# chenxing1999/recsys-benchmark

Hardware: AMD Instinct MI355X
Metric: samples/sec fwd+bwd, Criteo-26field DeepFM b=4096; HBM GB/s vs roofline (higher is better)
Workload: dtype f32; 1 GPU; C2 DeepFM Criteo-26field full embedding: F=26, D=16, N=33762577 rows, MLP 400x3+BN+dropout0.5, B=4096/GPU, fwd+bwd, 16 distinct uniform-id batches rotated (fresh ids every step), row-form (COO) table grads, criterion evaluated in the head launch (model(x, labels=y)), next batch known one step ahead (its table rows touched by riders of the weight-gradient launch), tables stored as one packed [N,32]; global_batch=4096, parallelism=single

## Files before the change

### recsys-benchmark_amd/csrc/tail.hip

```cpp
#include <cstdlib>
#include <type_traits>

#include "common.hpp"
#include "tail_gemm.hpp"
#include "tail_masks.hpp"

namespace {
using namespace mi;
using namespace tg;

__device__ __forceinline__ Drop make_drop(const uint8_t *bits, float p, int ld) {
  Drop d;
  d.bits = p > 0.f ? bits : nullptr;
  d.inv_keep = p > 0.f ? 1.f / (1.f - p) : 1.f;
  d.ld = ld;
  return d;
}

__global__ __launch_bounds__(kBlock) void k_tail_dropmask(MaskJob j, const int64_t *seed, float4 *__restrict__ zero4, int64_t nzero4) {
  mask_blocks(j, seed, zero4, nzero4, blockIdx.x, gridDim.x);
}

constexpr int kTilePitch = BNT + 4;
__device__ __forceinline__ void acc_to_lds(const floatx4 (&acc)[NSUB], const floatx4 (&accg)[NGRP], Cover cv, float *T, int wave,
// ... 473 lines not shown
  const float rstd = rsqrtf(var + eps);
  mu[n] = mean_a;
  sc[n] = gm * rstd;
  be[n] = bt;
  rstd_out[n] = rstd;
  if (running_mean) {
    running_mean[n] = (1.f - momentum) * rm + momentum * (mean_a + mo);
    const float unb = M > 1 ? m2_a / (float)(M - 1) : var;
    running_var[n] = (1.f - momentum) * rv + momentum * unb;
  }
}

template <bool MERGE>
__global__ __launch_bounds__(kBlock) void k_tail_head_fwd(ActDesc x, const float *__restrict__ w, const float *__restrict__ b,
                                                          const float *__restrict__ add, float *__restrict__ out, int M,
                                                          int N, BnFwd bn, int64_t *bump) {
  __shared__ __attribute__((aligned(16))) float cst[MERGE ? 3 * kCstPitch : 4];
  if (bump && blockIdx.x == 0 && threadIdx.x == 0) bump[0] += 1;
  const int lane = threadIdx.x & 63;
  const int wave0 = blockIdx.x * kWavesPerBlock + (threadIdx.x >> 6), nw = gridDim.x * kWavesPerBlock;
  const float bv = b ? b[0] : 0.f;
  auto rows = [&](const auto &act, const auto &between) {
    if (N <= 512) {
      const int c0 = lane * 4, c1 = lane * 4 + 256;
      const bool v0 = c0 < N, v1 = c1 < N;
      const float4 w0 = v0 ? ld4(w + c0) : make_float4(0.f, 0.f, 0.f, 0.f), w1 = v1 ? ld4(w + c1) : make_float4(0.f, 0.f, 0.f, 0.f);
      bool first = true;
      for (int m0 = wave0; m0 < M || first; m0 += 4 * nw) {
        typename std::remove_reference<decltype(act)>::type::Raw r0[4], r1[4];
        if (m0 < M) {
#pragma unroll
          for (int u = 0; u < 4; ++u) {
            const int m = min(m0 + u * nw, M - 1);
            if (v0) r0[u] = act.fetch(m, c0);
            if (v1) r1[u] = act.fetch(m, c1);
          }
        }
        if (first) between();
        first = false;
        if (m0 >= M) break;
#pragma unroll
        for (int u = 0; u < 4; ++u) {
          const int m = m0 + u * nw;
          if (m >= M) break;
          float s = 0.f;
          if (v0) { const float4 a = act.finish(r0[u], act.consts(c0), m, c0); s += a.x * w0.x + a.y * w0.y + a.z * w0.z + a.w * w0.w; }
          if (v1) { const float4 a = act.finish(r1[u], act.consts(c1), m, c1); s += a.x * w1.x + a.y * w1.y + a.z * w1.z + a.w * w1.w; }
          s = wave_sum(s);
          if (lane == 0) out[m] = s + bv + (add ? add[m] : 0.f);
        }
      }
      return;
    }
    between();
    for (int m = wave0; m < M; m += nw) {
      float s = 0.f;
      for (int c = lane * 4; c < N; c += 256) {
        const float4 a = act.finish(act.fetch(m, c), act.consts(c), m, c), ww = ld4(w + c);
        s += a.x * ww.x + a.y * ww.y + a.z * ww.z + a.w * ww.w;
      }
      s = wave_sum(s);
      if (lane == 0) out[m] = s + bv + (add ? add[m] : 0.f);
    }
  };
  const LoadAct act = make_act(x);
  if constexpr (MERGE) {
    const lds_cfp c = as_lds(cst);
    rows(LoadActL{x.Z, x.ld, c, c + kCstPitch, c + 2 * kCstPitch, act.drop}, [&]() {
      bn_merge_fwd<kBlock>(bn, M, N, cst, blockIdx.x == 0, (int)threadIdx.x);
      __syncthreads();
    });
  } else {
    rows(act, []() {});
  }
}

constexpr int kHeadRows = 8;
__global__ __launch_bounds__(kBlock) void k_tail_head_bwd(ActDesc x, const float *__restrict__ g, const float *__restrict__ w,
                                                          float *__restrict__ DY, float *__restrict__ part,
                                                          float *__restrict__ wpart, int M, int N, int reps) {
  const Drop drop = make_drop(x.keep, x.p, x.ld);
  const int c = threadIdx.x * 4;
  const bool cv = c < N;
  float4 s_dy = zero4(), s_dyz = zero4(), s_ga = zero4();
  float s_g = 0.f;
  float4 u_ = zero4(), sc = zero4(), be = zero4(), ww = zero4();
  if (cv) { u_ = ld4(x.mu + c); sc = ld4(x.sc + c); be = ld4(x.be + c); ww = ld4(w + c); }
  const int rows_per = (M + gridDim.x - 1) / gridDim.x;
  const int mb = blockIdx.x * rows_per, me = min(M, mb + rows_per);
  for (int m4 = mb; m4 < me; m4 += kHeadRows) {
    float4 z[kHeadRows];
    uint32_t kb[kHeadRows];
    float gv[kHeadRows];
#pragma unroll
    for (int u = 0; u < kHeadRows; ++u) {
      const int m = min(m4 + u, me - 1);
      gv[u] = g[m];
      if (cv) {
        z[u] = ld4(x.Z + (int64_t)m * x.ld + c);
        kb[u] = drop.fetch(m, c);
      }
    }
    loads_landed();
#pragma unroll
    for (int u = 0; u < kHeadRows; ++u) {
      const int m = m4 + u;
      if (m >= me) break;
      const float gm = gv[u];
      s_g += gm;
      if (!cv) continue;
      const float4 k = drop.scale4(kb[u], c);
      const float4 zc = make_float4(z[u].x - u_.x, z[u].y - u_.y, z[u].z - u_.z, z[u].w - u_.w);
      const float4 pre = make_float4(fmaf(zc.x, sc.x, be.x), fmaf(zc.y, sc.y, be.y), fmaf(zc.z, sc.z, be.z), fmaf(zc.w, sc.w, be.w));
      float4 dy;
      dy.x = pre.x > 0.f ? gm * ww.x * k.x : 0.f;
      dy.y = pre.y > 0.f ? gm * ww.y * k.y : 0.f;
      dy.z = pre.z > 0.f ? gm * ww.z * k.z : 0.f;
      dy.w = pre.w > 0.f ? gm * ww.w * k.w : 0.f;
      st4(DY + (int64_t)m * x.ld + c, dy);
      s_dy.x += dy.x; s_dy.y += dy.y; s_dy.z += dy.z; s_dy.w += dy.w;
      s_dyz.x += dy.x * zc.x; s_dyz.y += dy.y * zc.y; s_dyz.z += dy.z * zc.z; s_dyz.w += dy.w * zc.w;
      s_ga.x += gm * fmaxf(pre.x, 0.f) * k.x; s_ga.y += gm * fmaxf(pre.y, 0.f) * k.y;
      s_ga.z += gm * fmaxf(pre.z, 0.f) * k.z; s_ga.w += gm * fmaxf(pre.w, 0.f) * k.w;
    }
  }
  if (reps > 0) {
    __shared__ float sp[2 * 4 * kBlock + 4 * kBlock + 4];
    float *sw = sp + 2 * 4 * kBlock;
    if (cv) {
      st4(sp + c * 2, make_float4(s_dy.x, s_dyz.x, s_dy.y, s_dyz.y));
      st4(sp + c * 2 + 4, make_float4(s_dy.z, s_dyz.z, s_dy.w, s_dyz.w));
      st4(sw + c, s_ga);
    }
    if (threadIdx.x == 0) sw[N] = s_g;
    lds_barrier();
    const int rr = blockIdx.x % reps;
    float *o = part + (int64_t)rr * N * 2;
    for (int i = threadIdx.x; i < 2 * N; i += kBlock) atomicAdd(o + i, sp[i]);
    float *q = wpart + (int64_t)rr * (N + 4);
    for (int i = threadIdx.x; i <= N; i += kBlock) atomicAdd(q + i, sw[i]);
    return;
  }
  if (cv) {
    float *o = part + ((int64_t)blockIdx.x * N + c) * 2;
    st4(o, make_float4(s_dy.x, s_dyz.x, s_dy.y, s_dyz.y));
    st4(o + 4, make_float4(s_dy.z, s_dyz.z, s_dy.w, s_dyz.w));
    st4(wpart + (int64_t)blockIdx.x * (N + 4) + c, s_ga);
  }
  if (threadIdx.x == 0) wpart[(int64_t)blockIdx.x * (N + 4) + N] = s_g;
}

constexpr int kHeadLossCols = 512;
constexpr int kHeadLossRed = 3 * kHeadLossCols + 4;
template <int MERGE>
__global__ __launch_bounds__(kBlock) void k_tail_head_bce(ActDesc x, const float *__restrict__ w, const float *__restrict__ b,
                                                          const float *__restrict__ add, const float *__restrict__ y,
                                                          float *__restrict__ out, float *__restrict__ gout,
                                                          float *__restrict__ DY, float *__restrict__ part,
                                                          float *__restrict__ wpart, float *__restrict__ loss_ws, int M,
                                                          int N, BnFwd bn, int reps, int64_t *bump,
                                                          const float *__restrict__ upstream) {
  __shared__ __attribute__((aligned(16))) float cst[MERGE != 0 ? 3 * kCstPitch : 4];
  __shared__ __attribute__((aligned(16))) float red[kWavesPerBlock][kHeadLossRed];
  if (bump && blockIdx.x == 0 && threadIdx.x == 0) bump[0] += 1;
  const int lane = threadIdx.x & 63, wv = __builtin_amdgcn_readfirstlane(threadIdx.x >> 6);
  const int wave0 = blockIdx.x * kWavesPerBlock + wv, nw = gridDim.x * kWavesPerBlock;
  const Drop drop = make_drop(x.keep, x.p, x.ld);
  const float bv = b ? b[0] : 0.f;
  const float inv_m = 1.f / (float)M;
  const float gsc = upstream ? upstream[0] * inv_m : inv_m;
  const int c0 = lane * 4, c1 = lane * 4 + 256;
  const bool v0 = c0 < N, v1 = c1 < N;
  const float4 w0 = v0 ? ld4(w + c0) : zero4(), w1 = v1 ? ld4(w + c1) : zero4();
  float4 mu0 = zero4(), sc0 = zero4(), be0 = zero4(), mu1 = zero4(), sc1 = zero4(), be1 = zero4();
  float4 dy0 = zero4(), dz0 = zero4(), ga0 = zero4(), dy1 = zero4(), dz1 = zero4(), ga1 = zero4();
  float s_g = 0.f, s_loss = 0.f;
  bool first = true;
  for (int m0 = wave0; m0 < M || first; m0 += 4 * nw) {
    float4 z0[4], z1[4];
    uint32_t k0[4], k1[4];
    float av[4], yv[4];
    if (m0 < M) {
#pragma unroll
      for (int u = 0; u < 4; ++u) {
        const int m = min(m0 + u * nw, M - 1);
        if (v0) { z0[u] = ld4(x.Z + (int64_t)m * x.ld + c0); k0[u] = drop.fetch(m, c0); }
        if (v1) { z1[u] = ld4(x.Z + (int64_t)m * x.ld + c1); k1[u] = drop.fetch(m, c1); }
        av[u] = add ? add[m] : 0.f;
        yv[u] = y[m];
      }
    }
    if (first) {
      if constexpr (MERGE != 0) {
        if constexpr (MERGE == 2) bn_derive_fwd<kBlock>(bn, M, N, cst, blockIdx.x == 0, (int)threadIdx.x);
        else bn_merge_fwd<kBlock>(bn, M, N, cst, blockIdx.x == 0, (int)threadIdx.x);
        __syncthreads();
        const lds_cfp c = as_lds(cst);
        if (v0) { mu0 = vld4(c + c0); sc0 = vld4(c + kCstPitch + c0); be0 = vld4(c + 2 * kCstPitch + c0); }
        if (v1) { mu1 = vld4(c + c1); sc1 = vld4(c + kCstPitch + c1); be1 = vld4(c + 2 * kCstPitch + c1); }
      } else {
        if (v0) { mu0 = ld4(x.mu + c0); sc0 = ld4(x.sc + c0); be0 = ld4(x.be + c0); }
        if (v1) { mu1 = ld4(x.mu + c1); sc1 = ld4(x.sc + c1); be1 = ld4(x.be + c1); }
      }
    }
    first = false;
    loads_landed();
    if (m0 >= M) break;
    float sa[4];
    auto row0 = [&](int u, float4 &zc, float4 &pre, float4 &kk) {
      kk = drop.scale4(k0[u], c0);
      zc = make_float4(z0[u].x - mu0.x, z0[u].y - mu0.y, z0[u].z - mu0.z, z0[u].w - mu0.w);
      pre = make_float4(fmaf(zc.x, sc0.x, be0.x), fmaf(zc.y, sc0.y, be0.y), fmaf(zc.z, sc0.z, be0.z), fmaf(zc.w, sc0.w, be0.w));
    };
    auto row1 = [&](int u, float4 &zc, float4 &pre, float4 &kk) {
      kk = drop.scale4(k1[u], c1);
      zc = make_float4(z1[u].x - mu1.x, z1[u].y - mu1.y, z1[u].z - mu1.z, z1[u].w - mu1.w);
      pre = make_float4(fmaf(zc.x, sc1.x, be1.x), fmaf(zc.y, sc1.y, be1.y), fmaf(zc.z, sc1.z, be1.z), fmaf(zc.w, sc1.w, be1.w));
    };
#pragma unroll
    for (int u = 0; u < 4; ++u) {
      float4 zc, pre, kk;
      float s = 0.f;
      if (v0) {
        row0(u, zc, pre, kk);
        s += fmaxf(pre.x, 0.f) * kk.x * w0.x + fmaxf(pre.y, 0.f) * kk.y * w0.y + fmaxf(pre.z, 0.f) * kk.z * w0.z +
             fmaxf(pre.w, 0.f) * kk.w * w0.w;
      }
      if (v1) {
        row1(u, zc, pre, kk);
        s += fmaxf(pre.x, 0.f) * kk.x * w1.x + fmaxf(pre.y, 0.f) * kk.y * w1.y + fmaxf(pre.z, 0.f) * kk.z * w1.z +
             fmaxf(pre.w, 0.f) * kk.w * w1.w;
      }
      sa[u] = s;
    }
#pragma unroll
    for (int msk = 32; msk >= 1; msk >>= 1) {
#pragma unroll
      for (int u = 0; u < 4; ++u) sa[u] += __shfl_xor(sa[u], msk);
    }
    float4 d0[4], d1[4];
    float xo[4], go[4];
#pragma unroll
    for (int u = 0; u < 4; ++u) {
      const int m = m0 + u * nw;
      if (m >= M) break;
      float4 zc0 = zero4(), zc1 = zero4(), pre0 = zero4(), pre1 = zero4(), kk0 = zero4(), kk1 = zero4();
      if (v0) row0(u, zc0, pre0, kk0);
      if (v1) row1(u, zc1, pre1, kk1);
      const float s = sa[u];
      const float xl = s + bv + av[u];
      const float gm = gsc * (1.f / (1.f + expf(-xl)) - yv[u]);
      s_loss += fmaxf(xl, 0.f) - xl * yv[u] + log1pf(expf(-fabsf(xl)));
      s_g += gm;
      xo[u] = xl; go[u] = gm;
      if (v0) {
        float4 d;
        d.x = pre0.x > 0.f ? gm * w0.x * kk0.x : 0.f;
        d.y = pre0.y > 0.f ? gm * w0.y * kk0.y : 0.f;
        d.z = pre0.z > 0.f ? gm * w0.z * kk0.z : 0.f;
        d.w = pre0.w > 0.f ? gm * w0.w * kk0.w : 0.f;
        d0[u] = d;
        dy0.x += d.x; dy0.y += d.y; dy0.z += d.z; dy0.w += d.w;
        dz0.x += d.x * zc0.x; dz0.y += d.y * zc0.y; dz0.z += d.z * zc0.z; dz0.w += d.w * zc0.w;
        ga0.x += gm * fmaxf(pre0.x, 0.f) * kk0.x; ga0.y += gm * fmaxf(pre0.y, 0.f) * kk0.y;
        ga0.z += gm * fmaxf(pre0.z, 0.f) * kk0.z; ga0.w += gm * fmaxf(pre0.w, 0.f) * kk0.w;
      }
      if (v1) {
        float4 d;
        d.x = pre1.x > 0.f ? gm * w1.x * kk1.x : 0.f;
        d.y = pre1.y > 0.f ? gm * w1.y * kk1.y : 0.f;
        d.z = pre1.z > 0.f ? gm * w1.z * kk1.z : 0.f;
        d.w = pre1.w > 0.f ? gm * w1.w * kk1.w : 0.f;
        d1[u] = d;
        dy1.x += d.x; dy1.y += d.y; dy1.z += d.z; dy1.w += d.w;
        dz1.x += d.x * zc1.x; dz1.y += d.y * zc1.y; dz1.z += d.z * zc1.z; dz1.w += d.w * zc1.w;
        ga1.x += gm * fmaxf(pre1.x, 0.f) * kk1.x; ga1.y += gm * fmaxf(pre1.y, 0.f) * kk1.y;
        ga1.z += gm * fmaxf(pre1.z, 0.f) * kk1.z; ga1.w += gm * fmaxf(pre1.w, 0.f) * kk1.w;
      }
    }
#pragma unroll
    for (int u = 0; u < 4; ++u) {
      const int m = m0 + u * nw;
      if (m >= M) break;
      if (lane == 0) { out[m] = xo[u]; gout[m] = go[u]; }
      if (v0) st4(DY + (int64_t)m * x.ld + c0, d0[u]);
      if (v1) st4(DY + (int64_t)m * x.ld + c1, d1[u]);
    }
  }
  float *rp = red[wv];
  if (v0) {
    st4(rp + 2 * c0, make_float4(dy0.x, dz0.x, dy0.y, dz0.y));
    st4(rp + 2 * c0 + 4, make_float4(dy0.z, dz0.z, dy0.w, dz0.w));
    st4(rp + 2 * kHeadLossCols + c0, ga0);
  }
  if (v1) {
    st4(rp + 2 * c1, make_float4(dy1.x, dz1.x, dy1.y, dz1.y));
    st4(rp + 2 * c1 + 4, make_float4(dy1.z, dz1.z, dy1.w, dz1.w));
    st4(rp + 2 * kHeadLossCols + c1, ga1);
  }
  if (lane == 0) { rp[3 * kHeadLossCols] = s_g; rp[3 * kHeadLossCols + 1] = s_loss; }
  lds_barrier();
  const int rr = blockIdx.x % reps;
  constexpr int kSumThreads = kBlock - kWave;
  if (wv < kWavesPerBlock - 1) {
    float *o = part + (int64_t)rr * N * 2;
    for (int i = threadIdx.x; i < 2 * N; i += kSumThreads) atomicAdd(o + i, (red[0][i] + red[1][i]) + (red[2][i] + red[3][i]));
    float *q = wpart + (int64_t)rr * (N + 4);
    for (int i = threadIdx.x; i <= N; i += kSumThreads) {
      const int j = i < N ? 2 * kHeadLossCols + i : 3 * kHeadLossCols;
      atomicAdd(q + i, (red[0][j] + red[1][j]) + (red[2][j] + red[3][j]));
    }
  } else {
    if (lane == 0) {
      const int j = 3 * kHeadLossCols + 1;
      const float lp = ((red[0][j] + red[1][j]) + (red[2][j] + red[3][j])) * inv_m;
      atomicAdd(loss_ws + 4 + rr, lp);
      __threadfence();
      const uint32_t mine = ((uint32_t)gridDim.x - (uint32_t)rr + (uint32_t)reps - 1u) / (uint32_t)reps;
      const uint32_t old = atomicAdd(reinterpret_cast<uint32_t *>(loss_ws + 4 + reps) + rr, 1u);
      if (old == mine - 1u) {
        __threadfence();
        const float v = __hip_atomic_load(loss_ws + 4 + rr, __ATOMIC_RELAXED, __HIP_MEMORY_SCOPE_AGENT);
        atomicAdd(loss_ws, v);
      }
    }
    loads_landed();
  }
}

__global__ __launch_bounds__(kBlock) void k_bn_finalize_bwd(const float *__restrict__ part, int nblk, int M, int N,
                                                            const float *__restrict__ gamma, const float *__restrict__ rstd,
                                                            float *__restrict__ dgamma, float *__restrict__ dbeta,
                                                            float *__restrict__ al, float *__restrict__ bz,
                                                            float *__restrict__ de, const float *__restrict__ wpart,
                                                            int nwblk, float *__restrict__ dw, float *__restrict__ db,
                                                            int affine, float *__restrict__ dbias, float *__restrict__ db2) {
  __shared__ float sh[kFinGroups][kFinCols][3];
  const int cl = threadIdx.x % kFinCols, grp = threadIdx.x / kFinCols;
  const int n = blockIdx.x * kFinCols + cl;
  float r = 0.f, gm = 1.f;
  if (grp == 0 && n < N) { r = rstd[n]; if (gamma) gm = gamma[n]; }
  float s1 = 0.f, s2 = 0.f, sw = 0.f;
  if (n < N) {
    const int per = (nblk + kFinGroups - 1) / kFinGroups, t0 = grp * per, t1 = min(nblk, t0 + per);
    for (int base = t0; base < t1; base += 16) {
      float2 v[16];
#pragma unroll
      for (int u = 0; u < 16; ++u) v[u] = *reinterpret_cast<const float2 *>(part + ((int64_t)min(base + u, t1 - 1) * N + n) * 2);
#pragma unroll
      for (int u = 0; u < 16; ++u)
        if (base + u < t1) { s1 += v[u].x; s2 += v[u].y; }
    }
  }
  if (wpart && n <= N) {
    const int per = (nwblk + kFinGroups - 1) / kFinGroups, t0 = grp * per, t1 = min(nwblk, t0 + per);
    for (int base = t0; base < t1; base += 16) {
      float v[16];
#pragma unroll
      for (int u = 0; u < 16; ++u) v[u] = wpart[(int64_t)min(base + u, t1 - 1) * (N + 4) + n];
#pragma unroll
      for (int u = 0; u < 16; ++u)
        if (base + u < t1) sw += v[u];
    }
  }
  sh[grp][cl][0] = s1; sh[grp][cl][1] = s2; sh[grp][cl][2] = sw;
  __syncthreads();
  if (grp != 0 || n > N) return;
  s1 = 0.f; s2 = 0.f; sw = 0.f;
#pragma unroll
  for (int q = 0; q < kFinGroups; ++q) { s1 += sh[q][cl][0]; s2 += sh[q][cl][1]; sw += sh[q][cl][2]; }
  if (wpart) {
    if (n < N) dw[n] = sw;
    else {
      if (db) db[0] = sw;
      if (db2) db2[0] = sw;
    }
  }
  if (n >= N) return;
  const float dg = s2 * r;
  if (dgamma) dgamma[n] = dg;
  if (dbeta) dbeta[n] = s1;
  const float inv_m = 1.f / (float)M;
  al[n] = gm * r;
  bz[n] = affine ? 0.f : -gm * r * r * dg * inv_m;
  de[n] = affine ? 0.f : -gm * r * s1 * inv_m;
  if (affine && dbias) dbias[n] = gm * r * s1;
}

__global__ __launch_bounds__(kBlock) void k_tail_affine_consts(AffineJob j) {
  affine_consts_blocks(j, (int)blockIdx.x, (int)gridDim.x);
}

struct DgradArgs {
  DzDesc dz;
  const float *W;
  int ldw;
  ActDesc prev;
  float *OUT;
  int ldo;
  float *part;
  int part_rep;
  float *dz_out;
  int M, N, K;
  int ncols, ntn;
  BnBwd bn;
  const float *fm_emb;
  const float *fm_sum;
  const float *fm_gy;
  float *fm_g1;
  int fm_D;
  const int64_t *fm_slot;
  int fm_pitch;
};

template <bool DZ, bool MID, bool MERGE, bool FM = false>
__global__ __launch_bounds__(kThreads) void k_tail_dgrad(DgradArgs a) {
  __shared__ __attribute__((aligned(16))) float lds[kLdsFloats + (MERGE ? kCstFloats : 0)];
  const int mt_total = (a.M + BM - 1) / BM;
  const int tile = xcd_logical(blockIdx.x, mt_total * a.ntn);
  if (tile < 0) return;

  const int mt = tile / a.ntn, nt = tile % a.ntn;
  const int m0 = mt * BM, k0 = nt * a.ncols;
  const int rows_valid = min(BM, a.M - m0), cols_valid = min(a.ncols, a.K - k0);
  const int lane = threadIdx.x & 63, wave = threadIdx.x >> 6;
  floatx4 acc[NSUB], accg[NGRP];
#pragma unroll
  for (int s = 0; s < NSUB; ++s) acc[s] = floatx4{0.f, 0.f, 0.f, 0.f};
#pragma unroll
  for (int q = 0; q < NGRP; ++q) accg[q] = floatx4{0.f, 0.f, 0.f, 0.f};
  Cover cv{NSUB, 0};

  const LoadDz dzl = make_dz(a.dz);
  const LoadPlain dyp{a.dz.DY, a.dz.ld};
  const LoadPlain wp{a.W, a.ldw};
  const OtOperand<BNT, LoadPlain> opC{wp, k0, cols_valid, a.N};
  if constexpr (MERGE) {
    const lds_cfp c = as_lds(lds + kLdsFloats);
    const LoadDzL dzm{a.dz.DY, a.dz.Z, a.dz.ld, c, c + kCstPitch, c + 2 * kCstPitch, c + 3 * kCstPitch};
    float *cst = lds + kLdsFloats;
    const bool writer = tile == 0, wwriter = tile == min(1, mt_total * a.ntn - 1);
    cv = main_loop_cover(acc, accg, cols_valid, lds, 0, a.N, KcOperand<64, Tee<LoadDzL>>{Tee<LoadDzL>{dzm, nt == 0 ? a.dz_out : nullptr, a.dz.ld}, m0, rows_valid, a.N}, opC,
                    make_pre([&]() { bn_merge_bwd<kThreads - kProd>(a.bn, a.M, a.N, cst, writer, wwriter, (int)threadIdx.x); }));
  } else if constexpr (DZ)
    cv = main_loop_cover(acc, accg, cols_valid, lds, 0, a.N, KcOperand<64, Tee<LoadDz>>{Tee<LoadDz>{dzl, nt == 0 ? a.dz_out : nullptr, a.dz.ld}, m0, rows_valid, a.N}, opC);
  else cv = main_loop_cover(acc, accg, cols_valid, lds, 0, a.N, KcOperand<64, LoadPlain>{dyp, m0, rows_valid, a.N}, opC);

  float *T = lds;
  acc_to_lds(acc, accg, cv, T, wave, lane);
  if constexpr (FM) lds_barrier();
  else __syncthreads();
  const int t = threadIdx.x;
  if constexpr (FM) {
    static_assert(!MID, "the FM epilogue belongs to the product whose output is the tail's input gradient");
    float4 e[4], sm[4], da[4];
    float gy[4];
    int64_t sl[4];
    bool ok[4];
#pragma unroll
    for (int k = 0; k < 4; ++k) {
      const int i = t + k * kThreads, row = i / 28, c = (i % 28) * 4;
      ok[k] = i < 64 * 28 && row < rows_valid && c < cols_valid;
      const int m = m0 + (ok[k] ? row : 0), kc = k0 + (ok[k] ? c : 0);
      e[k] = ld4(a.fm_emb + (int64_t)m * a.K + kc);
      sm[k] = ld4(a.fm_sum + (int64_t)m * a.fm_D + kc % a.fm_D);
      gy[k] = a.fm_gy[m];
      da[k] = ld4(T + (ok[k] ? row : 0) * kTilePitch + (ok[k] ? c : 0));
      if (a.fm_slot) sl[k] = a.fm_slot[(int64_t)m * (a.K / a.fm_D) + kc / a.fm_D];
    }
    const bool g1w = a.fm_g1 && nt == 0;
    const int F = a.K / a.fm_D, ng1 = rows_valid * F;
    float g1v[4];
// ... 246 lines not shown
    tiles = mt * a.ntn;
    if (x_mu) MI_LAUNCH("tail_fwd_gemm_small", (k_tail_fwd<true, false, false, 2>), grid8(tiles), kThreads, stream, a);
    else MI_LAUNCH("tail_fwd_gemm_small", (k_tail_fwd<false, false, false, 2>), grid8(tiles), kThreads, stream, a);
    return launch_status();
  }

  if (x_stats) MI_LAUNCH("tail_fwd_gemm", (k_tail_fwd<true, true>), grid8(tiles), kThreads, stream, a);
  else if (x_mu && dma) MI_LAUNCH("tail_fwd_gemm", (k_tail_fwd<true, false, true>), grid8(tiles), kThreads, stream, a);
  else if (x_mu) MI_LAUNCH("tail_fwd_gemm", (k_tail_fwd<true, false>), grid8(tiles), kThreads, stream, a);
  else if (dma) MI_LAUNCH("tail_fwd_gemm", (k_tail_fwd<false, false, true>), grid8(tiles), kThreads, stream, a);
  else MI_LAUNCH("tail_fwd_gemm", (k_tail_fwd<false, false>), grid8(tiles), kThreads, stream, a);
  return launch_status();
}

int mi_tail_fwd_gemm(const float *X, int32_t ldx, const float *x_mu, const float *x_sc, const float *x_be, float x_p,
                     const uint8_t *x_keep, const float *W, int32_t ldw, float *Z, int32_t ldz, float *part, float *a_out,
                     int32_t M, int32_t N, int32_t K, void *stream) {
  return mi_tail_fwd_gemm_m(X, ldx, x_mu, x_sc, x_be, x_p, x_keep, W, ldw, Z, ldz, part, a_out, M, N, K, nullptr, stream);
}

int mi_tail_dropout_masks_z(const int64_t *seed, int32_t nlayers, const int64_t *salts, const float *ps, const int32_t *lds,
                            uint8_t *const *bits, int32_t M, float *zero_buf, int64_t zero_floats, void *stream) {
  MaskJob j;
  int64_t grid;
  const int rc = mask_job(seed, nlayers, salts, ps, lds, bits, M, zero_buf, zero_floats, j, &grid);
  if (rc != MI_OK || grid == 0) return rc;
  MI_LAUNCH("tail_dropout_masks", k_tail_dropmask, (int)grid, kBlock, stream, j, seed, reinterpret_cast<float4 *>(zero_buf),
            zero_floats / 4);
  return launch_status();
}

int mi_tail_dropout_masks(const int64_t *seed, int32_t nlayers, const int64_t *salts, const float *ps, const int32_t *lds,
                          uint8_t *const *bits, int32_t M, void *stream) {
  return mi_tail_dropout_masks_z(seed, nlayers, salts, ps, lds, bits, M, nullptr, 0, stream);
}

int64_t mi_tail_part_elems(int32_t M, int32_t N) { return (int64_t)((M + BM - 1) / BM) * N * 2; }

int mi_tail_bn_finalize_fwd(const float *part, int32_t M, int32_t N, const float *gamma, const float *beta,
                            const float *mean_offset, float *running_mean, float *running_var, float momentum, float eps,
                            int64_t *num_batches_tracked, int64_t *seed_bump, float *mu, float *sc, float *be, float *rstd,
                            void *stream) {
  return mi_tail_bn_finalize_fwd_r(part, M, N, gamma, beta, mean_offset, running_mean, running_var, momentum, eps,
                                   num_batches_tracked, seed_bump, mu, sc, be, rstd, nullptr, stream);
}

int mi_tail_bn_finalize_fwd_r(const float *part, int32_t M, int32_t N, const float *gamma, const float *beta,
                              const float *mean_offset, float *running_mean, float *running_var, float momentum, float eps,
                              int64_t *num_batches_tracked, int64_t *seed_bump, float *mu, float *sc, float *be, float *rstd,
                              const mi_tail_mask_ride *ride, void *stream) {
  if (M <= 0 || N <= 0 || !part || !mu || !sc || !be || !rstd) return MI_ERR_INVALID_ARG;
  const int nfin = (N + kFinCols - 1) / kFinCols;
  MaskRide r;
  r.j.n = 0; r.seed = nullptr; r.zero4 = nullptr; r.nzero4 = 0;
  r.mask_blocks = 0; r.aff.nl = 0;
  int64_t extra = 0;
  if (ride) {
    if (seed_bump && seed_bump == ride->seed) return MI_ERR_INVALID_ARG;
    const int rc = mask_job(ride->seed, ride->nlayers, ride->salts, ride->ps, ride->lds, ride->bits, ride->M, ride->zero_buf,
                            ride->zero_floats, r.j, &extra);
    if (rc != MI_OK) return rc;
    r.seed = ride->seed;
    r.zero4 = reinterpret_cast<float4 *>(ride->zero_buf);
    r.nzero4 = ride->zero_floats / 4;
  }
  if (extra > 0) {
    MI_LAUNCH("tail_bn_finalize_fwd_ride", k_bn_finalize_fwd<true>, nfin + (int)extra, kBlock, stream, part, M, N, gamma, beta,
              mean_offset, running_mean, running_var, momentum, eps, num_batches_tracked, seed_bump, mu, sc, be, rstd, r);
  } else {
    MI_LAUNCH("tail_bn_finalize_fwd", k_bn_finalize_fwd<false>, nfin, kBlock, stream, part, M, N, gamma, beta,
              mean_offset, running_mean, running_var, momentum, eps, num_batches_tracked, seed_bump, mu, sc, be, rstd, r);
  }
  return launch_status();
}

int mi_tail_head_fwd_m(const float *Z, int32_t ldz, const float *mu, const float *sc, const float *be, float p,
                       const uint8_t *keep, const float *w, const float *b, const float *add, float *out, int32_t M,
                       int32_t N, const mi_tail_bn_fwd *stats, void *stream) {
  if (M < 0 || N <= 0) return MI_ERR_INVALID_ARG;
  if (M == 0) return MI_OK;
  BnFwd bn{};
  int64_t *bump = nullptr;
  if (stats && !stats->part) {
    bump = stats->seed_bump;
    stats = nullptr;
  }
  if (stats) {
    if (N > kCstPitch) return MI_ERR_UNSUPPORTED;
    if (!bn_fwd_view(stats, &bn)) return MI_ERR_INVALID_ARG;
    mu = stats->mu; sc = stats->sc; be = stats->be;
  }
  if (!Z || !mu || !sc || !be || !w || !out) return MI_ERR_INVALID_ARG;
  if (!vec_ok(Z, ldz) || N % 4 || !aligned16(w)) return MI_ERR_UNSUPPORTED;
  if (p > 0.f && (!keep || ldz % 8)) return MI_ERR_INVALID_ARG;
  const ActDesc x{Z, ldz, mu, sc, be, p, keep};
  if (stats) {
    const int per_cu = (M + kWavesPerBlock - 1) / kWavesPerBlock < 256 ? (M + kWavesPerBlock - 1) / kWavesPerBlock : 256;
    const int grid = per_cu;
    MI_LAUNCH("tail_head_fwd", (k_tail_head_fwd<true>), grid, kBlock, stream, x, w, b, add, out, M, N, bn, (int64_t *)nullptr);
  } else {
    MI_LAUNCH("tail_head_fwd", (k_tail_head_fwd<false>), grid_for_waves(M), kBlock, stream, x, w, b, add, out, M, N, bn, bump);
  }
  return launch_status();
}

int mi_tail_head_fwd(const float *Z, int32_t ldz, const float *mu, const float *sc, const float *be, float p,
                     const uint8_t *keep, const float *w, const float *b, const float *add, float *out, int32_t M,
                     int32_t N, void *stream) {
  return mi_tail_head_fwd_m(Z, ldz, mu, sc, be, p, keep, w, b, add, out, M, N, nullptr, stream);
}

int32_t mi_tail_head_blocks(int32_t M) { return M >= 64 * 256 ? 256 : (M + 15) / 16 > 0 ? (M + 15) / 16 : 1; }

int mi_tail_head_bwd(const float *Z, int32_t ldz, const float *mu, const float *sc, const float *be, float p,
                     const uint8_t *keep, const float *g, const float *w, float *DY, float *part, float *wpart,
                     int32_t M, int32_t N, void *stream) {
  return mi_tail_head_bwd_s(Z, ldz, mu, sc, be, p, keep, g, w, DY, part, wpart, 0, M, N, stream);
}

int mi_tail_head_bwd_s(const float *Z, int32_t ldz, const float *mu, const float *sc, const float *be, float p,
                       const uint8_t *keep, const float *g, const float *w, float *DY, float *part, float *wpart,
                       int32_t sum_reps, int32_t M, int32_t N, void *stream) {
  if (M <= 0 || N <= 0 || sum_reps < 0 || sum_reps > 64) return MI_ERR_INVALID_ARG;
  if (!Z || !mu || !sc || !be || !g || !w || !DY || !part || !wpart) return MI_ERR_INVALID_ARG;
  if (!vec_ok(Z, ldz) || N % 4 || N > 4 * kBlock || !aligned16(w) || !aligned16(DY)) return MI_ERR_UNSUPPORTED;
  if (p > 0.f && (!keep || ldz % 8)) return MI_ERR_INVALID_ARG;
  const ActDesc x{Z, ldz, mu, sc, be, p, keep};
  MI_LAUNCH("tail_head_bwd", k_tail_head_bwd, mi_tail_head_blocks(M), kBlock, stream, x, g, w, DY, part, wpart, M, N, sum_reps);
  return launch_status();
}

int32_t mi_tail_head_bce_ws_elems(int32_t sum_reps) { return sum_reps > 0 ? (4 + 2 * sum_reps + 3) / 4 * 4 : 0; }

int mi_tail_head_bce(const float *Z, int32_t ldz, const float *mu, const float *sc, const float *be, float p,
                     const uint8_t *keep, const float *w, const float *b, const float *add, const float *y, float *out,
                     float *g, float *DY, float *part, float *wpart, int32_t sum_reps, float *loss_ws, int32_t M, int32_t N,
                     const mi_tail_bn_fwd *stats, const float *upstream, void *stream) {
  if (M <= 0 || N <= 0 || sum_reps <= 0 || sum_reps > 64) return MI_ERR_INVALID_ARG;
  BnFwd bn{};
  int64_t *bump = nullptr;
  if (stats && !stats->part) {
    bump = stats->seed_bump;
    stats = nullptr;
  }
  if (stats) {
    if (!bn_fwd_view(stats, &bn)) return MI_ERR_INVALID_ARG;
    mu = stats->mu; sc = stats->sc; be = stats->be;
  }
  if (!Z || !mu || !sc || !be || !w || !y || !out || !g || !DY || !part || !wpart || !loss_ws) return MI_ERR_INVALID_ARG;
  if (!vec_ok(Z, ldz) || N % 4 || N > kHeadLossCols || !aligned16(w) || !aligned16(DY)) return MI_ERR_UNSUPPORTED;
  if (p > 0.f && (!keep || ldz % 8)) return MI_ERR_INVALID_ARG;
  const ActDesc x{Z, ldz, mu, sc, be, p, keep};
  const int waves = (M + 3) / 4;
  const int grid = (waves + kWavesPerBlock - 1) / kWavesPerBlock < 256 ? (waves + kWavesPerBlock - 1) / kWavesPerBlock : 256;
  if (stats && bn.nrep > 0)
    MI_LAUNCH("tail_head_bce", (k_tail_head_bce<2>), grid, kBlock, stream, x, w, b, add, y, out, g, DY, part, wpart, loss_ws, M,
              N, bn, sum_reps, (int64_t *)nullptr, upstream);
  else if (stats)
    MI_LAUNCH("tail_head_bce", (k_tail_head_bce<1>), grid, kBlock, stream, x, w, b, add, y, out, g, DY, part, wpart, loss_ws, M,
              N, bn, sum_reps, (int64_t *)nullptr, upstream);
  else
    MI_LAUNCH("tail_head_bce", (k_tail_head_bce<0>), grid, kBlock, stream, x, w, b, add, y, out, g, DY, part, wpart, loss_ws,
              M, N, bn, sum_reps, bump, upstream);
  return launch_status();
}

int mi_tail_bn_finalize_bwd(const float *part, int32_t nblk, int32_t M, int32_t N, const float *gamma, const float *rstd,
                            float *dgamma, float *dbeta, float *al, float *bz, float *de, const float *wpart,
                            int32_t nwblk, float *dw, float *db, void *stream) {
  return mi_tail_bn_finalize_bwd_a(part, nblk, M, N, gamma, rstd, dgamma, dbeta, al, bz, de, wpart, nwblk, dw, db, 0, nullptr,
                                   stream);
}

int mi_tail_bn_finalize_bwd_a(const float *part, int32_t nblk, int32_t M, int32_t N, const float *gamma, const float *rstd,
                              float *dgamma, float *dbeta, float *al, float *bz, float *de, const float *wpart,
                              int32_t nwblk, float *dw, float *db, int32_t affine, float *dbias, void *stream) {
  return mi_tail_bn_finalize_bwd_b(part, nblk, M, N, gamma, rstd, dgamma, dbeta, al, bz, de, wpart, nwblk, dw, db, affine, dbias,
                                   nullptr, stream);
}

int mi_tail_bn_finalize_bwd_b(const float *part, int32_t nblk, int32_t M, int32_t N, const float *gamma, const float *rstd,
                              float *dgamma, float *dbeta, float *al, float *bz, float *de, const float *wpart,
                              int32_t nwblk, float *dw, float *db, int32_t affine, float *dbias, float *db2, void *stream) {
  if (M <= 0 || N <= 0 || nblk <= 0 || !part || !rstd || !al || !bz || !de) return MI_ERR_INVALID_ARG;
  if (wpart && !dw) return MI_ERR_INVALID_ARG;
  MI_LAUNCH("tail_bn_finalize_bwd", k_bn_finalize_bwd, (N + 1 + kFinCols - 1) / kFinCols, kBlock, stream, part, nblk, M, N,
            gamma, rstd, dgamma, dbeta, al, bz, de, wpart, nwblk, dw, db, affine, dbias, db2);
  return launch_status();
}

int mi_tail_affine_consts(int32_t nlayers, const int32_t *widths, const float *const *gamma, const float *const *beta,
                          const float *const *running_mean, const float *const *running_var, const float *const *bias,
                          const float *eps, float *const *mu, float *const *sc, float *const *be, float *const *rstd,
                          void *stream) {
  AffineJob j;
  int blocks = 0;
  const int rc = affine_job(nlayers, widths, gamma, beta, running_mean, running_var, bias, eps, mu, sc, be, rstd, j, &blocks);
  if (rc != MI_OK || blocks == 0) return rc;
  MI_LAUNCH("tail_affine_consts", k_tail_affine_consts, blocks, kBlock, stream, j);
  return launch_status();
}

static int dgrad_launch(const float *DY, const float *Zl, int32_t ld, const float *mu, const float *al, const float *bz,
                        const float *de, const float *W, int32_t ldw, const float *pZ, int32_t pld, const float *p_mu,
                        const float *p_sc, const float *p_be, float p_p, const uint8_t *p_keep, float *OUT, int32_t ldo,
                        float *part, float *dz_out, int32_t M, int32_t N, int32_t K, const mi_tail_bn_bwd *sums,
                        const float *fm_emb, const float *fm_sum, const float *fm_gy, float *fm_g1, int32_t fm_D,
                        int32_t part_reps, void *stream, const int64_t *fm_slot = nullptr);

int mi_tail_dgrad_gemm_m(const float *DY, const float *Zl, int32_t ld, const float *mu, const float *al, const float *bz,
                         const float *de, const float *W, int32_t ldw, const float *pZ, int32_t pld, const float *p_mu,
                         const float *p_sc, const float *p_be, float p_p, const uint8_t *p_keep, float *OUT, int32_t ldo,
                         float *part, float *dz_out, int32_t M, int32_t N, int32_t K, const mi_tail_bn_bwd *sums,
                         void *stream) {
  return dgrad_launch(DY, Zl, ld, mu, al, bz, de, W, ldw, pZ, pld, p_mu, p_sc, p_be, p_p, p_keep, OUT, ldo, part, dz_out, M, N,
                      K, sums, nullptr, nullptr, nullptr, nullptr, 0, 0, stream);
}

int mi_tail_dgrad_gemm_s(const float *DY, const float *Zl, int32_t ld, const float *mu, const float *al, const float *bz,
                         const float *de, const float *W, int32_t ldw, const float *pZ, int32_t pld, const float *p_mu,
                         const float *p_sc, const float *p_be, float p_p, const uint8_t *p_keep, float *OUT, int32_t ldo,
                         float *part, int32_t part_reps, float *dz_out, int32_t M, int32_t N, int32_t K,
                         const mi_tail_bn_bwd *sums, void *stream) {
  if (part_reps < 0 || part_reps > 64 || (part_reps > 0 && !part)) return MI_ERR_INVALID_ARG;
  return dgrad_launch(DY, Zl, ld, mu, al, bz, de, W, ldw, pZ, pld, p_mu, p_sc, p_be, p_p, p_keep, OUT, ldo, part, dz_out, M, N,
                      K, sums, nullptr, nullptr, nullptr, nullptr, 0, part_reps, stream);
}

int mi_tail_dgrad_gemm_fm(const float *DY, const float *Zl, int32_t ld, const float *mu, const float *al, const float *bz,
                          const float *de, const float *W, int32_t ldw, float *gvals, float *dz_out, int32_t M, int32_t N,
                          int32_t K, const mi_tail_bn_bwd *sums, const float *emb, const float *emb_sum, const float *g_y,
                          float *g1vals, int32_t D, void *stream) {
  if (!emb || !emb_sum || !g_y || D <= 0 || D % 4 || K % D) return MI_ERR_INVALID_ARG;
  if (!aligned16(emb) || !aligned16(emb_sum)) return MI_ERR_UNSUPPORTED;
  return dgrad_launch(DY, Zl, ld, mu, al, bz, de, W, ldw, nullptr, K, nullptr, nullptr, nullptr, 0.f, nullptr, gvals, K,
                      nullptr, dz_out, M, N, K, sums, emb, emb_sum, g_y, g1vals, D, 0, stream);
}

int mi_tail_dgrad_gemm_fm_slot(const float *DY, const float *Zl, int32_t ld, const float *mu, const float *al, const float *bz,
                               const float *de, const float *W, int32_t ldw, float *gbuf, float *dz_out, int32_t M, int32_t N,
                               int32_t K, const mi_tail_bn_bwd *sums, const float *emb, const float *emb_sum, const float *g_y,
                               const int64_t *slot, int32_t D, void *stream) {
  if (!emb || !emb_sum || !g_y || !slot || !gbuf || D <= 0 || D % 4 || K % D) return MI_ERR_INVALID_ARG;
  if (!aligned16(emb) || !aligned16(emb_sum) || !aligned16(gbuf)) return MI_ERR_UNSUPPORTED;
  return dgrad_launch(DY, Zl, ld, mu, al, bz, de, W, ldw, nullptr, K, nullptr, nullptr, nullptr, 0.f, nullptr, gbuf, D + 4,
                      nullptr, dz_out, M, N, K, sums, emb, emb_sum, g_y, nullptr, D, 0, stream, slot);
}

static int dgrad_launch(const float *DY, const float *Zl, int32_t ld, const float *mu, const float *al, const float *bz,
                        const float *de, const float *W, int32_t ldw, const float *pZ, int32_t pld, const float *p_mu,
                        const float *p_sc, const float *p_be, float p_p, const uint8_t *p_keep, float *OUT, int32_t ldo,
                        float *part, float *dz_out, int32_t M, int32_t N, int32_t K, const mi_tail_bn_bwd *sums,
                        const float *fm_emb, const float *fm_sum, const float *fm_gy, float *fm_g1, int32_t fm_D,
                        int32_t part_reps, void *stream, const int64_t *fm_slot) {
  if (M < 0 || N <= 0 || K <= 0) return MI_ERR_INVALID_ARG;
  if (M == 0) return MI_OK;
  if (!DY || !W || !OUT) return MI_ERR_INVALID_ARG;
  DgradArgs a;
  a.part_rep = part_reps;
  a.fm_emb = fm_emb; a.fm_sum = fm_sum; a.fm_gy = fm_gy; a.fm_g1 = fm_g1; a.fm_D = fm_D;
  a.fm_slot = fm_slot; a.fm_pitch = fm_D + 4;
  a.bn = BnBwd{};
  if (sums) {
    if (N > kCstPitch) return MI_ERR_UNSUPPORTED;
    if (!sums->part || !aligned16(sums->part) || sums->nblk <= 0 || !sums->rstd || !sums->al || !sums->bz || !sums->de || !mu || !Zl) return MI_ERR_INVALID_ARG;
    if (sums->wpart && (!sums->dw || sums->nwblk <= 0)) return MI_ERR_INVALID_ARG;
    a.bn = BnBwd{sums->part, sums->nblk, sums->gamma, sums->rstd, mu, sums->dgamma, sums->dbeta, sums->al, sums->bz, sums->de,
                 sums->wpart, sums->nwblk, sums->dw, sums->db, sums->db2, sums->affine, sums->dbias};
    al = sums->al; bz = sums->bz; de = sums->de;
  }
  if (al && (!Zl || !mu || !bz || !de)) return MI_ERR_INVALID_ARG;
  if (p_mu && (!pZ || !p_sc || !p_be)) return MI_ERR_INVALID_ARG;
  if (!vec_ok(DY, ld) || !vec_ok(W, ldw) || !vec_ok(OUT, ldo) || N % 4 || K % 4 || (pZ && !vec_ok(pZ, pld)))
    return MI_ERR_UNSUPPORTED;
  a.dz = DzDesc{DY, Zl, ld, mu, al, bz, de};
  a.W = W; a.ldw = ldw;
  if (p_mu && p_p > 0.f && (!p_keep || pld % 8)) return MI_ERR_INVALID_ARG;
  a.prev = ActDesc{pZ, pld, p_mu, p_sc, p_be, p_p, p_keep};
  a.OUT = OUT; a.ldo = ldo; a.part = part;
  if (dz_out && (!al || !aligned16(dz_out))) return MI_ERR_INVALID_ARG;
  a.dz_out = dz_out;
  a.M = M; a.N = N; a.K = K;
  a.ncols = cols_per_tile(K, &a.ntn);
  const int tiles = ((M + BM - 1) / BM) * a.ntn;
  const bool dz = al != nullptr, mid = p_mu != nullptr;
  if (fm_emb) {
    if (mid) return MI_ERR_INVALID_ARG;
    if (sums) MI_LAUNCH("tail_dgrad_gemm_fm", (k_tail_dgrad<true, false, true, true>), grid8(tiles), kThreads, stream, a);
    else if (dz) MI_LAUNCH("tail_dgrad_gemm_fm", (k_tail_dgrad<true, false, false, true>), grid8(tiles), kThreads, stream, a);
    else MI_LAUNCH("tail_dgrad_gemm_fm", (k_tail_dgrad<false, false, false, true>), grid8(tiles), kThreads, stream, a);
    return launch_status();
  }
  if (sums && mid) MI_LAUNCH("tail_dgrad_gemm", (k_tail_dgrad<true, true, true>), grid8(tiles), kThreads, stream, a);
  else if (sums) MI_LAUNCH("tail_dgrad_gemm", (k_tail_dgrad<true, false, true>), grid8(tiles), kThreads, stream, a);
  else if (dz && mid) MI_LAUNCH("tail_dgrad_gemm", (k_tail_dgrad<true, true, false>), grid8(tiles), kThreads, stream, a);
  else if (dz) MI_LAUNCH("tail_dgrad_gemm", (k_tail_dgrad<true, false, false>), grid8(tiles), kThreads, stream, a);
  else if (mid) MI_LAUNCH("tail_dgrad_gemm", (k_tail_dgrad<false, true, false>), grid8(tiles), kThreads, stream, a);
  else MI_LAUNCH("tail_dgrad_gemm", (k_tail_dgrad<false, false, false>), grid8(tiles), kThreads, stream, a);
  return launch_status();
}

int mi_tail_dgrad_gemm(const float *DY, const float *Zl, int32_t ld, const float *mu, const float *al, const float *bz,
                       const float *de, const float *W, int32_t ldw, const float *pZ, int32_t pld, const float *p_mu,
                       const float *p_sc, const float *p_be, float p_p, const uint8_t *p_keep, float *OUT, int32_t ldo,
                       float *part, float *dz_out, int32_t M, int32_t N, int32_t K, void *stream) {
  return mi_tail_dgrad_gemm_m(DY, Zl, ld, mu, al, bz, de, W, ldw, pZ, pld, p_mu, p_sc, p_be, p_p, p_keep, OUT, ldo, part,
                              dz_out, M, N, K, nullptr, stream);
}

int32_t mi_tail_wgrad_splits(int32_t M, int32_t N, int32_t K) {
  int ntk;
  cols_per_tile(K, &ntk);
  const int tiles = ((N + 63) / 64) * ntk;
  int s = 256 / (tiles > 0 ? tiles : 1);
  const int max_s = (M + BK - 1) / BK;
// ... 35 lines not shown
```

Before: 19.15 million samples/s.

## Split head BCE rows across 8 waves per block and issue loss atomics early

The head BCE kernel gets a wave-count template parameter. The MERGE=2 and MERGE=0 variants launch 8 waves per block, each owning 2 of the 16 rows per trip, so per-wave register arrays halve and more waves hide latency over the same grid. The loss partial and its completion-counter atomic now run inside the last loop iteration through a small LDS reduction, so they overlap the final stores instead of trailing the column reduction. The costs are a larger LDS reduction buffer, an extra barrier, and more complex per-wave trip bookkeeping.

```diff
diff --git a/recsys-benchmark_amd/csrc/tail.hip b/recsys-benchmark_amd/csrc/tail.hip
--- a/recsys-benchmark_amd/csrc/tail.hip
+++ b/recsys-benchmark_amd/csrc/tail.hip
@@ -649,19 +649,33 @@
 
 constexpr int kHeadLossCols = 512;
 constexpr int kHeadLossRed = 3 * kHeadLossCols + 4;
-template <int MERGE>
-__global__ __launch_bounds__(kBlock) void k_tail_head_bce(ActDesc x, const float *__restrict__ w, const float *__restrict__ b,
-                                                          const float *__restrict__ add, const float *__restrict__ y,
-                                                          float *__restrict__ out, float *__restrict__ gout,
-                                                          float *__restrict__ DY, float *__restrict__ part,
-                                                          float *__restrict__ wpart, float *__restrict__ loss_ws, int M,
-                                                          int N, BnFwd bn, int reps, int64_t *bump,
-                                                          const float *__restrict__ upstream) {
+constexpr int kHeadTripRows = 16;
+template <int NWV>
+__device__ __forceinline__ float head_red_sum(const float (*red)[kHeadLossRed], int i) {
+  const float a = (red[0][i] + red[1][i]) + (red[2][i] + red[3][i]);
+  if constexpr (NWV == 8) return a + ((red[4][i] + red[5][i]) + (red[6][i] + red[7][i]));
+  else return a;
+}
+template <int MERGE, int NWV>
+__global__ __launch_bounds__(NWV * kWave) void k_tail_head_bce(ActDesc x, const float *__restrict__ w, const float *__restrict__ b,
+                                                               const float *__restrict__ add, const float *__restrict__ y,
+                                                               float *__restrict__ out, float *__restrict__ gout,
+                                                               float *__restrict__ DY, float *__restrict__ part,
+                                                               float *__restrict__ wpart, float *__restrict__ loss_ws, int M,
+                                                               int N, BnFwd bn, int reps, int64_t *bump,
+                                                               const float *__restrict__ upstream) {
+  static_assert(NWV == 4 || NWV == 8, "a wave takes 4 or 2 of the trip's 16 rows");
+  constexpr int NT = NWV * kWave, R = kHeadTripRows / NWV;
   __shared__ __attribute__((aligned(16))) float cst[MERGE != 0 ? 3 * kCstPitch : 4];
-  __shared__ __attribute__((aligned(16))) float red[kWavesPerBlock][kHeadLossRed];
+  __shared__ __attribute__((aligned(16))) float red[NWV][kHeadLossRed];
+  __shared__ float lsh[NWV];
   if (bump && blockIdx.x == 0 && threadIdx.x == 0) bump[0] += 1;
   const int lane = threadIdx.x & 63, wv = __builtin_amdgcn_readfirstlane(threadIdx.x >> 6);
-  const int wave0 = blockIdx.x * kWavesPerBlock + wv, nw = gridDim.x * kWavesPerBlock;
+  const int nw = gridDim.x * 4, trip = 4 * nw;
+  const int wave0 = blockIdx.x * 4 + (wv & 3) + (wv >> 2) * R * nw;
+  const int T = (M - (int)blockIdx.x * 4 + trip - 1) / trip;
+  const bool chain = wv == NWV - 1;
+  uint32_t old = 0u;
   const Drop drop = make_drop(x.keep, x.p, x.ld);
   const float bv = b ? b[0] : 0.f;
   const float inv_m = 1.f / (float)M;
@@ -672,14 +686,16 @@
   float4 mu0 = zero4(), sc0 = zero4(), be0 = zero4(), mu1 = zero4(), sc1 = zero4(), be1 = zero4();
   float4 dy0 = zero4(), dz0 = zero4(), ga0 = zero4(), dy1 = zero4(), dz1 = zero4(), ga1 = zero4();
   float s_g = 0.f, s_loss = 0.f;
-  bool first = true;
-  for (int m0 = wave0; m0 < M || first; m0 += 4 * nw) {
-    float4 z0[4], z1[4];
-    uint32_t k0[4], k1[4];
-    float av[4], yv[4];
-    if (m0 < M) {
-#pragma unroll
-      for (int u = 0; u < 4; ++u) {
+  int t = 0;
+  do {
+    const int m0 = wave0 + t * trip;
+    const bool have = m0 < M;
+    float4 z0[R], z1[R];
+    uint32_t k0[R], k1[R];
+    float av[R], yv[R];
+    if (have) {
+#pragma unroll
+      for (int u = 0; u < R; ++u) {
         const int m = min(m0 + u * nw, M - 1);
         if (v0) { z0[u] = ld4(x.Z + (int64_t)m * x.ld + c0); k0[u] = drop.fetch(m, c0); }
         if (v1) { z1[u] = ld4(x.Z + (int64_t)m * x.ld + c1); k1[u] = drop.fetch(m, c1); }
@@ -687,10 +703,10 @@
         yv[u] = y[m];
       }
     }
-    if (first) {
+    if (t == 0) {
       if constexpr (MERGE != 0) {
-        if constexpr (MERGE == 2) bn_derive_fwd<kBlock>(bn, M, N, cst, blockIdx.x == 0, (int)threadIdx.x);
-        else bn_merge_fwd<kBlock>(bn, M, N, cst, blockIdx.x == 0, (int)threadIdx.x);
+        if constexpr (MERGE == 2) bn_derive_fwd<NT>(bn, M, N, cst, blockIdx.x == 0, (int)threadIdx.x);
+        else bn_merge_fwd<NT>(bn, M, N, cst, blockIdx.x == 0, (int)threadIdx.x);
         __syncthreads();
         const lds_cfp c = as_lds(cst);
         if (v0) { mu0 = vld4(c + c0); sc0 = vld4(c + kCstPitch + c0); be0 = vld4(c + 2 * kCstPitch + c0); }
@@ -700,10 +716,7 @@
         if (v1) { mu1 = ld4(x.mu + c1); sc1 = ld4(x.sc + c1); be1 = ld4(x.be + c1); }
       }
     }
-    first = false;
     loads_landed();
-    if (m0 >= M) break;
-    float sa[4];
     auto row0 = [&](int u, float4 &zc, float4 &pre, float4 &kk) {
       kk = drop.scale4(k0[u], c0);
       zc = make_float4(z0[u].x - mu0.x, z0[u].y - mu0.y, z0[u].z - mu0.z, z0[u].w - mu0.w);
@@ -714,42 +727,64 @@
       zc = make_float4(z1[u].x - mu1.x, z1[u].y - mu1.y, z1[u].z - mu1.z, z1[u].w - mu1.w);
       pre = make_float4(fmaf(zc.x, sc1.x, be1.x), fmaf(zc.y, sc1.y, be1.y), fmaf(zc.z, sc1.z, be1.z), fmaf(zc.w, sc1.w, be1.w));
     };
-#pragma unroll
-    for (int u = 0; u < 4; ++u) {
-      float4 zc, pre, kk;
-      float s = 0.f;
-      if (v0) {
-        row0(u, zc, pre, kk);
-        s += fmaxf(pre.x, 0.f) * kk.x * w0.x + fmaxf(pre.y, 0.f) * kk.y * w0.y + fmaxf(pre.z, 0.f) * kk.z * w0.z +
-             fmaxf(pre.w, 0.f) * kk.w * w0.w;
-      }
-      if (v1) {
-        row1(u, zc, pre, kk);
-        s += fmaxf(pre.x, 0.f) * kk.x * w1.x + fmaxf(pre.y, 0.f) * kk.y * w1.y + fmaxf(pre.z, 0.f) * kk.z * w1.z +
-             fmaxf(pre.w, 0.f) * kk.w * w1.w;
-      }
-      sa[u] = s;
-    }
-#pragma unroll
-    for (int msk = 32; msk >= 1; msk >>= 1) {
-#pragma unroll
-      for (int u = 0; u < 4; ++u) sa[u] += __shfl_xor(sa[u], msk);
-    }
-    float4 d0[4], d1[4];
-    float xo[4], go[4];
-#pragma unroll
-    for (int u = 0; u < 4; ++u) {
-      const int m = m0 + u * nw;
-      if (m >= M) break;
+    float xo[R], go[R];
+    if (have) {
+      float sa[R];
+#pragma unroll
+      for (int u = 0; u < R; ++u) {
+        float4 zc, pre, kk;
+        float s = 0.f;
+        if (v0) {
+          row0(u, zc, pre, kk);
+          s += fmaxf(pre.x, 0.f) * kk.x * w0.x + fmaxf(pre.y, 0.f) * kk.y * w0.y + fmaxf(pre.z, 0.f) * kk.z * w0.z +
+               fmaxf(pre.w, 0.f) * kk.w * w0.w;
+        }
+        if (v1) {
+          row1(u, zc, pre, kk);
+          s += fmaxf(pre.x, 0.f) * kk.x * w1.x + fmaxf(pre.y, 0.f) * kk.y * w1.y + fmaxf(pre.z, 0.f) * kk.z * w1.z +
+               fmaxf(pre.w, 0.f) * kk.w * w1.w;
+        }
+        sa[u] = s;
+      }
+#pragma unroll
+      for (int msk = 32; msk >= 1; msk >>= 1) {
+#pragma unroll
+        for (int u = 0; u < R; ++u) sa[u] += __shfl_xor(sa[u], msk);
+      }
+#pragma unroll
+      for (int u = 0; u < R; ++u) {
+        const float xl = sa[u] + bv + av[u];
+        const float gm = gsc * (1.f / (1.f + expf(-xl)) - yv[u]);
+        xo[u] = xl; go[u] = gm;
+        if (m0 + u * nw < M) {
+          s_loss += fmaxf(xl, 0.f) - xl * yv[u] + log1pf(expf(-fabsf(xl)));
+          s_g += gm;
+        }
+      }
+    }
+    if (t == T - 1) {
+      if (lane == 0) lsh[wv] = s_loss;
+      lds_barrier();
+      if (chain && lane == 0) {
+        float lp = (lsh[0] + lsh[1]) + (lsh[2] + lsh[3]);
+        if constexpr (NWV == 8) lp = ((lsh[0] + lsh[4]) + (lsh[1] + lsh[5])) + ((lsh[2] + lsh[6]) + (lsh[3] + lsh[7]));
+        const int rr = blockIdx.x % reps;
+        atomicAdd(loss_ws + 4 + rr, lp * inv_m);
+        __threadfence();
+        uint32_t zero = 0u;
+        asm volatile("" : "+v"(zero));
+        old = atomicAdd(reinterpret_cast<uint32_t *>(loss_ws + 4 + reps) + rr + zero, 1u);
+      }
+    }
+    if (!have) continue;
+    float4 d0[R], d1[R];
+#pragma unroll
+    for (int u = 0; u < R; ++u) {
+      if (m0 + u * nw >= M) continue;
       float4 zc0 = zero4(), zc1 = zero4(), pre0 = zero4(), pre1 = zero4(), kk0 = zero4(), kk1 = zero4();
       if (v0) row0(u, zc0, pre0, kk0);
       if (v1) row1(u, zc1, pre1, kk1);
-      const float s = sa[u];
-      const float xl = s + bv + av[u];
-      const float gm = gsc * (1.f / (1.f + expf(-xl)) - yv[u]);
-      s_loss += fmaxf(xl, 0.f) - xl * yv[u] + log1pf(expf(-fabsf(xl)));
-      s_g += gm;
-      xo[u] = xl; go[u] = gm;
+      const float gm = go[u];
       if (v0) {
         float4 d;
         d.x = pre0.x > 0.f ? gm * w0.x * kk0.x : 0.f;
@@ -776,14 +811,15 @@
       }
     }
 #pragma unroll
-    for (int u = 0; u < 4; ++u) {
+    for (int u = 0; u < R; ++u) {
       const int m = m0 + u * nw;
-      if (m >= M) break;
-      if (lane == 0) { out[m] = xo[u]; gout[m] = go[u]; }
-      if (v0) st4(DY + (int64_t)m * x.ld + c0, d0[u]);
-      if (v1) st4(DY + (int64_t)m * x.ld + c1, d1[u]);
-    }
-  }
+      if (m < M) {
+        if (lane == 0) { out[m] = xo[u]; gout[m] = go[u]; }
+        if (v0) st4(DY + (int64_t)m * x.ld + c0, d0[u]);
+        if (v1) st4(DY + (int64_t)m * x.ld + c1, d1[u]);
+      }
+    }
+  } while (++t < T);
   float *rp = red[wv];
   if (v0) {
     st4(rp + 2 * c0, make_float4(dy0.x, dz0.x, dy0.y, dz0.y));
@@ -795,26 +831,21 @@
     st4(rp + 2 * c1 + 4, make_float4(dy1.z, dz1.z, dy1.w, dz1.w));
     st4(rp + 2 * kHeadLossCols + c1, ga1);
   }
-  if (lane == 0) { rp[3 * kHeadLossCols] = s_g; rp[3 * kHeadLossCols + 1] = s_loss; }
+  if (lane == 0) rp[3 * kHeadLossCols] = s_g;
   lds_barrier();
   const int rr = blockIdx.x % reps;
-  constexpr int kSumThreads = kBlock - kWave;
-  if (wv < kWavesPerBlock - 1) {
+  constexpr int kSumThreads = NT - kWave;
+  if (!chain) {
     float *o = part + (int64_t)rr * N * 2;
-    for (int i = threadIdx.x; i < 2 * N; i += kSumThreads) atomicAdd(o + i, (red[0][i] + red[1][i]) + (red[2][i] + red[3][i]));
+    for (int i = threadIdx.x; i < 2 * N; i += kSumThreads) atomicAdd(o + i, head_red_sum<NWV>(red, i));
     float *q = wpart + (int64_t)rr * (N + 4);
     for (int i = threadIdx.x; i <= N; i += kSumThreads) {
       const int j = i < N ? 2 * kHeadLossCols + i : 3 * kHeadLossCols;
-      atomicAdd(q + i, (red[0][j] + red[1][j]) + (red[2][j] + red[3][j]));
+      atomicAdd(q + i, head_red_sum<NWV>(red, j));
     }
   } else {
     if (lane == 0) {
-      const int j = 3 * kHeadLossCols + 1;
-      const float lp = ((red[0][j] + red[1][j]) + (red[2][j] + red[3][j])) * inv_m;
-      atomicAdd(loss_ws + 4 + rr, lp);
-      __threadfence();
       const uint32_t mine = ((uint32_t)gridDim.x - (uint32_t)rr + (uint32_t)reps - 1u) / (uint32_t)reps;
-      const uint32_t old = atomicAdd(reinterpret_cast<uint32_t *>(loss_ws + 4 + reps) + rr, 1u);
       if (old == mine - 1u) {
         __threadfence();
         const float v = __hip_atomic_load(loss_ws + 4 + rr, __ATOMIC_RELAXED, __HIP_MEMORY_SCOPE_AGENT);
@@ -1367,15 +1398,15 @@
   if (p > 0.f && (!keep || ldz % 8)) return MI_ERR_INVALID_ARG;
   const ActDesc x{Z, ldz, mu, sc, be, p, keep};
   const int waves = (M + 3) / 4;
-  const int grid = (waves + kWavesPerBlock - 1) / kWavesPerBlock < 256 ? (waves + kWavesPerBlock - 1) / kWavesPerBlock : 256;
+  const int grid = (waves + 3) / 4 < 256 ? (waves + 3) / 4 : 256;
   if (stats && bn.nrep > 0)
-    MI_LAUNCH("tail_head_bce", (k_tail_head_bce<2>), grid, kBlock, stream, x, w, b, add, y, out, g, DY, part, wpart, loss_ws, M,
+    MI_LAUNCH("tail_head_bce", (k_tail_head_bce<2, 8>), grid, 8 * kWave, stream, x, w, b, add, y, out, g, DY, part, wpart, loss_ws, M,
               N, bn, sum_reps, (int64_t *)nullptr, upstream);
   else if (stats)
-    MI_LAUNCH("tail_head_bce", (k_tail_head_bce<1>), grid, kBlock, stream, x, w, b, add, y, out, g, DY, part, wpart, loss_ws, M,
+    MI_LAUNCH("tail_head_bce", (k_tail_head_bce<1, 4>), grid, 4 * kWave, stream, x, w, b, add, y, out, g, DY, part, wpart, loss_ws, M,
               N, bn, sum_reps, (int64_t *)nullptr, upstream);
   else
-    MI_LAUNCH("tail_head_bce", (k_tail_head_bce<0>), grid, kBlock, stream, x, w, b, add, y, out, g, DY, part, wpart, loss_ws,
+    MI_LAUNCH("tail_head_bce", (k_tail_head_bce<0, 8>), grid, 8 * kWave, stream, x, w, b, add, y, out, g, DY, part, wpart, loss_ws,
               M, N, bn, sum_reps, bump, upstream);
   return launch_status();
 }
```

Measured after the change: 19.28 million samples/s (median of 6 runs). Within noise of the previous version (+0.7%).
